# tzt101/MichiGAN

Measured on AMD Instinct MI355X. Metric: training images/sec at 512x512 (G+D step), higher is better.
Workload: dtype bf16; 1 GPU; SPADEB G + multiscale PatchGAN D + VGG19 + Gabor orientation losses, full G step + D step (Adam), bs=8/GPU, 512x512, BASELINE.json configs[2]; global_batch=8, batch_per_gpu=8, resolution=512, parallelism=dp1, init=reference default (xavier, 0.02), random VGG weights

## Files before the change

### michigan_amd/_cabi.py

```python
from __future__ import annotations

import contextlib
import ctypes
import os

MG_F32, MG_BF16 = 0, 1
MG_ACT_NONE, MG_ACT_RELU, MG_ACT_LRELU, MG_ACT_TANH = 0, 1, 2, 3
MG_EPI_PLAIN, MG_EPI_SPADE = 0, 1
MG_MAX_TAPS = 64
MG_ABI_VERSION = 10
MG_COMM_ID_BYTES = 128

OPT_CONV_BIGTILES, OPT_CONV_HALO, OPT_WGRAD3X3, OPT_CONV_HALO_BIG, OPT_CONV_SPLITK, OPT_CONV_THIN, OPT_CONV_WIDE, OPT_CONV_DOT = 1, 2, 3, 4, 5, 6, 7, 8
OPT_PROBE_HALO_VARIANT, OPT_PROBE_WGRAD3X3, OPT_PROBE_ADDR_LO, OPT_PROBE_ADDR_HI, OPT_PROBE_NOXPRE = 10, 12, 13, 14, 15
OPT_WGRAD_MIN_STAGES, OPT_NORM_BWD_VEC, OPT_PROBE_HALO_LDSPAD, OPT_CONV_HALO64, OPT_PROBE_HALO64_DBG, OPT_WGRAD3X3_STRIPE = 18, 19, 21, 22, 23, 24

_i32, _f32, _vp, _i64 = ctypes.c_int32, ctypes.c_float, ctypes.c_void_p, ctypes.c_int64


class ConvDesc(ctypes.Structure):
    _fields_ = [
        ("in_", _vp), ("wt", _vp), ("out", _vp), ("bias", _vp), ("resid", _vp), ("x", _vp),
        ("mean", _vp), ("rstd", _vp), ("gamma_out", _vp),
        ("dtype", _i32), ("N", _i32), ("Hin", _i32), ("Win", _i32), ("Cin", _i32),
# ... 102 lines not shown
    "mg_pixel_affine": ([_vp, _vp, _vp, _vp, _i32, _i64, _i32, _vp, _vp], _i32),
    "mg_bg_compose": ([_vp, _vp, _vp, _i64, _i32, _i32, _i32, _i32, _i32, _i32, _vp, _vp, _vp], _i32),
    "mg_masked_mean_fill": ([_vp, _vp, _vp, _vp, _i32, _i32, _i32, _i32, _vp, _vp], _i32),
    "mg_orient_loss_fwd": ([_vp, _vp, _vp, _i32, _i64, _vp, _i64, _i32, _i64, _vp, _vp, _vp], _i32),
    "mg_orient_loss_bwd": ([_vp, _vp, _vp, _i32, _i64, _vp, _i64, _vp, _vp, _vp, _i32, _i64, _vp, _vp], _i32),
    "mg_color_loss_fwd": ([_vp, _vp, _i64, _vp, _i64, _i32, _i32, _i32, _i32, _i32, _i32, _vp, _vp, _vp], _i32),
    "mg_color_loss_bwd": ([_vp, _vp, _i64, _vp, _i64, _vp, _vp, _vp, _i32, _i32, _i32, _i32, _i32, _i32, _vp, _vp], _i32),
    "mg_hair_lab_fwd": ([_vp, _vp, _i64, _vp, _i64, _vp, _i64, _vp, _i64, _vp, _i64, _i32, _i32, _i32, _i32, _i32, _i32, _vp, _vp, _vp, _vp], _i32),
    "mg_hair_lab_bwd": ([_vp, _vp, _i64, _vp, _i64, _vp, _i64, _vp, _vp, _vp, _i32, _i32, _i32, _i32, _i32, _i32, _vp, _vp], _i32),
    "mg_gabor_argmax_fwd": ([_vp, _vp, _vp, _vp, _i32, _i32, _i32, _i32, _i32, _vp], _i32),
    "mg_gabor_argmax_bwd": ([_vp, _vp, _vp, _vp, _i32, _i32, _i32, _i32, _i32, _vp], _i32),
    "mg_self_attention": ([_vp, _vp, _vp, _vp, _i32, _i32, _i32, _i32, _i32, _i64, _i64, _i64, _i64, _vp], _i32),
    "mg_sn_normalize": ([_vp, _i32, _f32, _vp, _vp, _vp, _vp], _i32),
    "mg_sn_scale": ([_vp, _vp, _vp, _i64, _vp], _i32),
    "mg_sn_bwd": ([_vp, _vp, _vp, _vp, _vp, _vp, _i32, _i32, _vp], _i32),
    "mg_adam_step": ([_vp, _vp, _vp, _vp, _i64, _f32, _f32, _f32, _f32, _i32, _f32, _vp], _i32),
    "mg_input_crop_u8": ([_vp, _vp, _vp, _vp, _vp, _vp, _i32, _i32, _i32, _i32, _i32, _i32, _i32, _i32, _vp], _i32),
    "mg_onehot_labels": ([_vp, _vp, _i32, _i64, _i32, _vp], _i32),
    "mg_orient_to_rgb_u8": ([_vp, _vp, _vp, _vp, _i64, _vp], _i32),
    "mg_generate_hole_u8": ([_vp, _vp, _vp, _vp, _vp, _vp, _i32, _i32, _i32, _vp], _i32),
    "mg_noise_octaves": ([_vp, _vp, _i32, _i32, _vp], _i32),
    "mg_resize_bicubic_u8": ([_vp, _vp, _vp, _vp, _vp, _i32, _vp, _vp, _i32, _i32, _i32, _i32, _i32, _i32, _i32, _vp], _i32),
    "mg_bicubic_ksize": ([_i32, _i32], _i32),
    "mg_inputs_set_option": ([_i32, _i32], _i32),
    "mg_bicubic_table": ([_i32, _i32, _vp, _vp], _i32),
    "mg_nearest_table": ([_i32, _i32, _vp], _i32),
    "mg_orient_rgb_table": ([_vp], _i32),
    "mg_noise_field_len": ([_i32], _i64),
    "mg_comm_unique_id": ([_vp], _i32),
    "mg_comm_init": ([_vp, _i32, _i32, ctypes.POINTER(_i64)], _i32),
    "mg_comm_destroy": ([_i64], _i32),
    "mg_comm_world": ([_i64, ctypes.POINTER(_i32), ctypes.POINTER(_i32)], _i32),
    "mg_allreduce_stats": ([_i64, _vp, _i64, _i32, _vp], _i32),
    "mg_allreduce_grads": ([_i64, _vp, _i64, _vp], _i32),
    "mg_probe_mfma_layout": ([_vp, _vp], _i32),
    "mg_probe_tr16": ([_vp, _vp, _vp], _i32),
    "mg_set_option": ([_i32, _i32], _i32),
    "mg_get_option": ([_i32, ctypes.POINTER(_i32)], _i32),
    "mg_sizeof_desc": ([_i32], _i32),
    "mg_abi_version": ([], _i32),
    "mg_last_error": ([], ctypes.c_char_p),
    "mg_feat_moment_workspace": ([_i32, _i64, _i32], _i64),
    "mg_feat_moment_loss_fwd": ([ctypes.POINTER(FeatMomentDesc), _vp], _i32),
    "mg_feat_moment_loss_bwd": ([ctypes.POINTER(FeatMomentDesc), _vp, _vp, _vp, _vp], _i32),
    "mg_orient_smooth": ([_vp, _vp, _vp, _vp, _vp, _vp, _vp, _i32, _i32, _i32, _vp], _i32),
    "mg_stroke_orient": ([_vp, _vp, _vp, _vp, _vp, _vp, _i32, _i32, _i32, _vp], _i32),
    "mg_stroke_compose": ([_vp, _vp, _vp, _vp, _vp, _vp, _vp, _i32, _i32, _i32, _i32, _i32, _i32, _vp, _vp], _i32),
    "mg_inpaint_finish": ([_vp, _vp, _vp, _vp, _vp, _vp, _i32, _i32, _i32, _i32, _i32, _vp, _vp, _vp], _i32),
}
_EDIT_PROTOS = {
    "mge_brush_u8": ([_vp, _vp, _i32, _i32, _i32, _i32, _vp], _i32),
    "mge_morph_u8": ([_vp, _vp, _i32, _i32, _i32, _i32, _i32, _vp, _i32, _i32, _i32, _vp], _i32),
}
EXPORTED_SYMBOLS = tuple(_PROTOS)
_NO_STATUS = {"mg_wgrad_det_workspace", "mg_norm_apply2_supported", "mg_grad_slot_blocks", "mg_pack_job_blocks", "mg_sn_layer_blocks", "mg_stats_workspace", "mg_sizeof_desc", "mg_abi_version", "mg_last_error", "mg_noise_field_len", "mg_bicubic_ksize",
              "mg_feat_moment_workspace"}
_BY_REF = {fn for fn, (argtypes, _) in _PROTOS.items()
           if argtypes and isinstance(getattr(argtypes[0], "_type_", None), type) and issubclass(argtypes[0]._type_, ctypes.Structure)}
DESC_MIRRORS = (ConvDesc, WgradDesc, GradSlot, PackJob, SnLayer, NormApply2Desc, PyramidDesc, FeatMomentDesc)

LIB_PATH = os.environ.get("MG_LIB") or os.path.join(os.path.dirname(os.path.abspath(__file__)), "lib", "libmichigan_hip.so")


class HipBackend:
    name = "hip"

    def __init__(self, path: str = LIB_PATH):
        if not os.path.exists(path) and path == LIB_PATH and os.environ.get("MG_AUTOBUILD", "1") != "0":
            import sys
            print("[michigan_amd] libmichigan_hip.so missing: building it with hipcc (gfx950), ~2 min", file=sys.stderr, flush=True)
            from . import build as _build
            _build.build_locked(verbose=False)
        if not os.path.exists(path):
            raise RuntimeError(
                f"libmichigan_hip.so not found at {path}: build it with "
                "`python -c 'import __graft_entry__ as g; g.build()'` (hipcc, gfx950). "
                "michigan_amd has no CPU / eager-PyTorch fallback.")
        import torch
        self._lib = ctypes.CDLL(path)
        for fn, (argtypes, restype) in list(_PROTOS.items()) + list(_EDIT_PROTOS.items()):
            f = getattr(self._lib, fn)
            f.argtypes, f.restype = argtypes, restype
        if self._lib.mg_abi_version() != MG_ABI_VERSION:
            raise RuntimeError("libmichigan_hip.so ABI version mismatch")
        if any(self._lib.mg_sizeof_desc(which) != ctypes.sizeof(mirror) for which, mirror in enumerate(DESC_MIRRORS)):
            raise RuntimeError("ctypes mirror of the descriptor structs is out of sync with include/michigan_hip.h")

    def __getattr__(self, fn):
        if fn not in _PROTOS and fn not in _EDIT_PROTOS:
            raise AttributeError(fn)
        raw = getattr(self._lib, fn)
        if fn in _NO_STATUS:
            return raw
        by_ref = fn in _BY_REF

        def call(*args):
            if by_ref:
                args = (ctypes.byref(args[0]),) + tuple(args[1:])
            rc = raw(*args)
            if rc != 0:
                msg = self._lib.mg_last_error()
                raise RuntimeError(f"{fn} failed (code {rc}): {msg.decode() if msg else '?'}")
            return rc
        self.__dict__[fn] = call
        return call


_backend = None


def backend():
    global _backend
    if _backend is None:
        _backend = HipBackend()
    return _backend


def set_backend(obj):
    global _backend
    prev, _backend = _backend, obj
    return prev


def get_option(key, be=None):
    v = _i32()
    (be or backend()).mg_get_option(key, ctypes.byref(v))
    return v.value


@contextlib.contextmanager
def options(values, be=None):
    be = be or backend()
    saved = {key: get_option(key, be) for key in values}
    try:
        for key, v in values.items():
            be.mg_set_option(key, v)
        yield
    finally:
        for key, v in saved.items():
            be.mg_set_option(key, v)
```

### michigan_amd/build.py

```python
from __future__ import annotations

import hashlib
import os
import shutil
import subprocess
import sys
from concurrent.futures import ThreadPoolExecutor

PKG_DIR = os.path.dirname(os.path.abspath(__file__))
REPO_ROOT = os.path.dirname(PKG_DIR)
CSRC = os.path.join(PKG_DIR, "csrc")
INCLUDE = os.path.join(REPO_ROOT, "include")
LIB_DIR = os.path.join(PKG_DIR, "lib")
OBJ_DIR = os.path.join(LIB_DIR, "obj")
LIB_PATH = os.path.join(LIB_DIR, "libmichigan_hip.so")

ARCH = "gfx950"
SOURCES = ["mg_api.hip", "mg_conv.hip", "mg_wgrad.hip", "mg_norm.hip", "mg_pointwise.hip", "mg_pack.hip", "mg_conv_halo.hip", "mg_conv_halo64.hip", "mg_gabor.hip", "mg_wgrad3x3.hip", "mg_spectral.hip", "mg_conv_thin.hip", "mg_inputs.hip", "mg_conv_dot.hip", "mg_loss.hip", "mg_grad.hip", "mg_weights.hip", "mg_glue.hip", "mg_color_loss.hip", "mg_hair_lab.hip", "mg_feat_moments.hip", "mg_orient_smooth.hip", "mg_stroke.hip", "mg_mask_edit.hip", "mg_attention.hip", "mg_comm.hip"]
CXXFLAGS = [f"--offload-arch={ARCH}", "-O3", "-std=c++17", "-fPIC", "-munsafe-fp-atomics",
            "-fno-gpu-rdc", f"-I{INCLUDE}", f"-I{CSRC}"]


def _hipcc() -> str:
    for cand in (os.environ.get("HIPCC"), "/opt/rocm/bin/hipcc", shutil.which("hipcc")):
        if cand and os.path.exists(cand):
            return cand
    raise RuntimeError("hipcc not found (looked at $HIPCC, /opt/rocm/bin/hipcc, PATH)")


def _public_headers() -> list:
    return sorted(os.path.join(d, f) for d, _, files in os.walk(INCLUDE) for f in files)


def _fingerprint(src: str = "") -> str:
    h = hashlib.sha256()
    h.update(" ".join(CXXFLAGS).encode())
    paths = [os.path.join(CSRC, f) for f in sorted(os.listdir(CSRC)) if f.endswith(".h") or (not src and f.endswith(".hip"))]
    paths += _public_headers()
    if src:
        paths.append(os.path.join(CSRC, src))
    for p in paths:
        if os.path.isfile(p):
            h.update(os.path.basename(p).encode())
            with open(p, "rb") as fh:
                h.update(fh.read())
    return h.hexdigest()


def source_hash() -> str:
    h = hashlib.sha256()
    h.update(" ".join(f for f in CXXFLAGS if not f.startswith("-I")).encode())
    for p in [os.path.join(CSRC, f) for f in sorted(os.listdir(CSRC))] + _public_headers():
        if p.endswith((".h", ".hip")):
            h.update(os.path.relpath(p, REPO_ROOT).replace(os.sep, "/").encode())
            with open(p, "rb") as fh:
                h.update(fh.read())
    return h.hexdigest()[:16]


def build(force: bool = False, verbose: bool = True) -> str:
    os.makedirs(OBJ_DIR, exist_ok=True)
    stamp = os.path.join(LIB_DIR, "build.stamp")
    fp = _fingerprint()
    if not force and os.path.exists(LIB_PATH) and os.path.exists(stamp):
        with open(stamp) as fh:
            if fh.read().strip() == fp:
                return LIB_PATH
    hipcc = _hipcc()

    def compile_one(src: str) -> str:
        obj = os.path.join(OBJ_DIR, os.path.splitext(src)[0] + ".o")
# ... 42 lines not shown
```

### michigan_amd/csrc/mg_pointwise.hip

```cpp
#include "mg_common.h"
#include "mg_launch.h"
#include "mg_reduce.h"

namespace {

template <typename T>
__global__ void act_bwd_kernel(const T* __restrict__ dy, const T* __restrict__ y, T* __restrict__ dpre,
                               int64_t nquads, int act, float slope)
{
    MG_GRID_STRIDE(i, nquads) {
        const f32x4_t d = ET<T>::load4(dy + i * 4), v = ET<T>::load4(y + i * 4);
        f32x4_t o;
#pragma unroll
        for (int j = 0; j < 4; ++j) o[j] = d[j] * mg_act_grad_from_out(v[j], act, slope);
        ET<T>::store4(dpre + i * 4, o);
    }
}

template <typename T>
__global__ void up2_fwd_kernel(const T* __restrict__ x, T* __restrict__ y, int N, int H, int W, int C)
{
    const int c4 = C / 4; const int Ho = 2 * H, Wo = 2 * W;
    const int64_t n = (int64_t)N * Ho * Wo * c4;
    MG_GRID_STRIDE(i, n) {
// ... 89 lines not shown
        const float inv = 1.f / (float)(pool_cnt(oy, H) * pool_cnt(ox, W));
#pragma unroll
        for (int j = 0; j < 4; ++j) s[j] *= inv;
        ET<T>::store4(y + i * 4, s);
    }
}
template <typename T>
__global__ void avgpool_bwd_kernel(const T* __restrict__ dy, T* __restrict__ dx, int N, int H, int W, int C, int Ho, int Wo)
{
    const int c4 = C / 4;
    const int64_t n = (int64_t)N * H * W * c4;
    MG_GRID_STRIDE(i, n) {
        const int qd = (int)(i % c4); int64_t p = i / c4;
        const int ix = (int)(p % W); p /= W;
        const int iy = (int)(p % H); const int b = (int)(p / H);
        f32x4_t s = {0.f, 0.f, 0.f, 0.f};
        for (int oy = (iy) >> 1; oy <= (iy + 1) >> 1; ++oy) {
            if (oy >= Ho) continue;
            for (int ox = (ix) >> 1; ox <= (ix + 1) >> 1; ++ox) {
                if (ox >= Wo) continue;
                const float inv = 1.f / (float)(pool_cnt(oy, H) * pool_cnt(ox, W));
                const f32x4_t v = ET<T>::load4(dy + (((size_t)b * Ho + oy) * Wo + ox) * C + qd * 4);
#pragma unroll
                for (int j = 0; j < 4; ++j) s[j] += v[j] * inv;
            }
        }
        ET<T>::store4(dx + i * 4, s);
    }
}

template <typename T>
__global__ void maxpool_fwd_kernel(const T* __restrict__ x, T* __restrict__ y, int N, int H, int W, int C, int Ho, int Wo)
{
    const int c4 = C / 4;
    const int64_t n = (int64_t)N * Ho * Wo * c4;
    MG_GRID_STRIDE(i, n) {
        const int qd = (int)(i % c4); int64_t p = i / c4;
        const int ox = (int)(p % Wo); p /= Wo;
        const int oy = (int)(p % Ho); const int b = (int)(p / Ho);
        const size_t base = (((size_t)b * H + 2 * oy) * W + 2 * ox) * C + qd * 4;
        const f32x4_t a = ET<T>::load4(x + base), bq = ET<T>::load4(x + base + C);
        const f32x4_t c = ET<T>::load4(x + base + (size_t)W * C), e = ET<T>::load4(x + base + (size_t)W * C + C);
        f32x4_t o;
#pragma unroll
        for (int j = 0; j < 4; ++j) o[j] = fmaxf(fmaxf(a[j], bq[j]), fmaxf(c[j], e[j]));
        ET<T>::store4(y + i * 4, o);
    }
}
template <typename T>
__global__ void maxpool_bwd_kernel(const T* __restrict__ dy, const T* __restrict__ x, T* __restrict__ dx,
                                   int N, int H, int W, int C, int Ho, int Wo, int relu_in)
{
    const int c4 = C / 4;
    const int64_t n = (int64_t)N * H * W * c4;
    MG_GRID_STRIDE(i, n) {
        const int qd = (int)(i % c4); int64_t p = i / c4;
        const int ix = (int)(p % W); p /= W;
        const int iy = (int)(p % H); const int b = (int)(p / H);
        const int oy = iy >> 1, ox = ix >> 1;
        f32x4_t o = {0.f, 0.f, 0.f, 0.f};
        if (oy < Ho && ox < Wo) {
            const size_t base = (((size_t)b * H + 2 * oy) * W + 2 * ox) * C + qd * 4;
            f32x4_t v[4];
            v[0] = ET<T>::load4(x + base); v[1] = ET<T>::load4(x + base + C);
            v[2] = ET<T>::load4(x + base + (size_t)W * C); v[3] = ET<T>::load4(x + base + (size_t)W * C + C);
            const f32x4_t g = ET<T>::load4(dy + (((size_t)b * Ho + oy) * Wo + ox) * C + qd * 4);
            const int me = (iy & 1) * 2 + (ix & 1);
#pragma unroll
            for (int j = 0; j < 4; ++j) {
                int arg = 0; float m = v[0][j];
#pragma unroll
                for (int k = 1; k < 4; ++k) if (v[k][j] > m) { m = v[k][j]; arg = k; }
                o[j] = (arg == me && (!relu_in || m > 0.f)) ? g[j] : 0.f;
            }
        }
        ET<T>::store4(dx + i * 4, o);
    }
}

template <typename T>
__global__ void blend_fwd_kernel(const T* __restrict__ bg, const T* __restrict__ x, const float* __restrict__ hair,
                                 const float* __restrict__ back, T* __restrict__ y, int64_t nquads, int C, int act, float slope)
{
    const int c4 = C / 4;
    MG_GRID_STRIDE(i, nquads) {
        const int64_t p = i / c4;
        const float wb = 1.f - hair[p], wx = 1.f - back[p];
        const f32x4_t b = ET<T>::load4(bg + i * 4), v = ET<T>::load4(x + i * 4);
        f32x4_t o;
#pragma unroll
        for (int j = 0; j < 4; ++j) o[j] = mg_act(b[j] * wb + v[j] * wx, act, slope);
        ET<T>::store4(y + i * 4, o);
    }
}
template <typename T>
__global__ void blend_bwd_kernel(const T* __restrict__ dy, const T* __restrict__ y, const float* __restrict__ hair,
                                 const float* __restrict__ back, T* __restrict__ dbg, T* __restrict__ dx, int64_t nquads, int C,
                                 int act, float slope)
{
    const int c4 = C / 4;
    MG_GRID_STRIDE(i, nquads) {
        const int64_t p = i / c4;
        const float wb = 1.f - hair[p], wx = 1.f - back[p];
        f32x4_t d = ET<T>::load4(dy + i * 4);
        if (act != MG_ACT_NONE) {
            const f32x4_t yv = ET<T>::load4(y + i * 4);
#pragma unroll
            for (int j = 0; j < 4; ++j) d[j] *= mg_act_grad_from_out(yv[j], act, slope);
        }
        f32x4_t a, b;
#pragma unroll
        for (int j = 0; j < 4; ++j) { a[j] = d[j] * wb; b[j] = d[j] * wx; }
        if (dbg) ET<T>::store4(dbg + i * 4, a);
        if (dx)  ET<T>::store4(dx + i * 4, b);
    }
}

__global__ void adam_kernel(float* __restrict__ p, const float* __restrict__ g, float* __restrict__ m, float* __restrict__ v,
                            int64_t n, float lr, float b1, float b2, float eps, float bc1, float bc2_sqrt, float gscale)
{
    MG_GRID_STRIDE(i, n) {
        const float gi = g[i] * gscale;
        const float w = 1.f - b1, mo = b1 == 0.f ? 0.f : m[i];
        const float mi = w < 0.5f ? mo + w * (gi - mo) : gi - (gi - mo) * (1.f - w);
        const float vi = v[i] * b2 + gi * gi * (1.f - b2);
        m[i] = mi; v[i] = vi;
        const float denom = sqrtf(vi) / bc2_sqrt + eps;
        p[i] = p[i] - (lr / bc1) * (mi / denom);
    }
// ... 189 lines not shown
        ET<T>::store4(out + (size_t)i * 8 + 4, b);
    }
}

extern "C" int mg_assemble_nhwc8(const float* planar, int32_t cp, const void* nhwc, int32_t cs, int32_t cf, void* out, int32_t dtype,
                                 int32_t N, int64_t HW, void* stream)
{
    MG_CHECK_ARG(out && (planar || cp == 0) && (nhwc || cf == 0), "mg_assemble_nhwc8: null pointer");
    MG_CHECK_ARG((dtype == MG_F32 || dtype == MG_BF16) && N > 0 && HW > 0 && cp >= 0 && cf >= 0 && cp + cf <= 8 && cf <= cs,
                 "mg_assemble_nhwc8: bad geometry (cp + cf <= 8, cf <= cs)");
    hipStream_t st = reinterpret_cast<hipStream_t>(stream);
    const int64_t npix = (int64_t)N * HW;
    mg_by_dtype(dtype, [&](auto t) { using T = typename decltype(t)::type;
        hipLaunchKernelGGL(assemble_nhwc8_kernel<T>, dim3(mg_ew_grid(npix, 8192)), dim3(MG_NTHR), 0, st, planar, cp, (const T*)nhwc, cs, cf, (T*)out, npix, HW); });
    MG_CHECK_LAUNCH("mg_assemble_nhwc8");
    return MG_OK;
}

template <typename T>
__global__ void grad_sum_act_kernel(const T* __restrict__ g1, const T* __restrict__ g2, const T* __restrict__ y, T* __restrict__ out,
                                    int64_t nquads, int act, float slope)
{
    MG_GRID_STRIDE(i, nquads) {
        f32x4_t a = ET<T>::load4(g1 + i * 4);
        if (g2) { const f32x4_t b = ET<T>::load4(g2 + i * 4);
#pragma unroll
            for (int j = 0; j < 4; ++j) a[j] += b[j]; }
        const f32x4_t v = ET<T>::load4(y + i * 4);
#pragma unroll
        for (int j = 0; j < 4; ++j) a[j] *= mg_act_grad_from_out(v[j], act, slope);
        ET<T>::store4(out + i * 4, a);
    }
}

extern "C" int mg_grad_sum_act(const void* g1, const void* g2, const void* y, void* out, int32_t dtype, int64_t numel, int32_t act,
                               float slope, void* stream)
{
    MG_CHECK_ARG(g1 && y && out, "mg_grad_sum_act: null pointer");
    MG_CHECK_ARG((dtype == MG_F32 || dtype == MG_BF16) && numel > 0 && (numel % 4) == 0, "mg_grad_sum_act: numel must be a positive multiple of 4");
    hipStream_t st = reinterpret_cast<hipStream_t>(stream);
    const int64_t nq = numel / 4;
    mg_by_dtype(dtype, [&](auto t) { using T = typename decltype(t)::type;
        hipLaunchKernelGGL(grad_sum_act_kernel<T>, dim3(mg_ew_grid(nq, 8192)), dim3(MG_NTHR), 0, st, (const T*)g1, (const T*)g2, (const T*)y, (T*)out, nq, act, slope); });
    MG_CHECK_LAUNCH("mg_grad_sum_act");
    return MG_OK;
}

extern "C" int mg_maxpool2_bwd(const void* dy, const void* x, void* dx, int32_t dtype, int32_t N, int32_t H, int32_t W, int32_t C, int32_t relu_input, void* stream)
{
    MG_EW_GEOM("mg_maxpool2_bwd"); MG_CHECK_ARG(dy && x && dx, "mg_maxpool2_bwd: null pointer");
    MG_CHECK_ARG(H >= 2 && W >= 2, "mg_maxpool2_bwd: H, W must be >= 2");
    hipStream_t st = reinterpret_cast<hipStream_t>(stream);
    const int Ho = H / 2, Wo = W / 2;
    const int g = mg_ew_grid((int64_t)N * H * W * (C / 4), 8192);
    mg_by_dtype(dtype, [&](auto t) { using T = typename decltype(t)::type;
        hipLaunchKernelGGL(maxpool_bwd_kernel<T>, dim3(g), dim3(MG_NTHR), 0, st, (const T*)dy, (const T*)x, (T*)dx, N, H, W, C, Ho, Wo, relu_input); });
    MG_CHECK_LAUNCH("mg_maxpool2_bwd");
    return MG_OK;
}

extern "C" int mg_blend_fwd(const void* bg, const void* x, const float* hair, const float* back, void* y,
                            int32_t dtype, int64_t P, int32_t C, int32_t act, float slope, void* stream)
{
    MG_CHECK_ARG(bg && x && hair && back && y, "mg_blend_fwd: null pointer");
    MG_CHECK_ARG((dtype == MG_F32 || dtype == MG_BF16) && P > 0 && C > 0 && (C % 4) == 0, "mg_blend_fwd: bad geometry");
    hipStream_t st = reinterpret_cast<hipStream_t>(stream);
    const int64_t nq = P * (C / 4);
    mg_by_dtype(dtype, [&](auto t) { using T = typename decltype(t)::type;
        hipLaunchKernelGGL(blend_fwd_kernel<T>, dim3(mg_ew_grid(nq, 8192)), dim3(MG_NTHR), 0, st, (const T*)bg, (const T*)x, hair, back, (T*)y, nq, C, act, slope); });
    MG_CHECK_LAUNCH("mg_blend_fwd");
    return MG_OK;
}
extern "C" int mg_blend_bwd(const void* dy, const void* y, const float* hair, const float* back, void* dbg, void* dx,
                            int32_t dtype, int64_t P, int32_t C, int32_t act, float slope, void* stream)
{
    MG_CHECK_ARG(dy && hair && back && (dbg || dx) && (y || act == MG_ACT_NONE), "mg_blend_bwd: null pointer");
    MG_CHECK_ARG((dtype == MG_F32 || dtype == MG_BF16) && P > 0 && C > 0 && (C % 4) == 0, "mg_blend_bwd: bad geometry");
    hipStream_t st = reinterpret_cast<hipStream_t>(stream);
    const int64_t nq = P * (C / 4);
    mg_by_dtype(dtype, [&](auto t) { using T = typename decltype(t)::type;
        hipLaunchKernelGGL(blend_bwd_kernel<T>, dim3(mg_ew_grid(nq, 8192)), dim3(MG_NTHR), 0, st, (const T*)dy, (const T*)y, hair, back, (T*)dbg, (T*)dx, nq, C, act, slope); });
    MG_CHECK_LAUNCH("mg_blend_bwd");
    return MG_OK;
}

extern "C" int mg_adam_step(float* param, const float* grad, float* exp_avg, float* exp_avg_sq,
                            int64_t numel, float lr, float beta1, float beta2, float eps, int32_t step,
                            float grad_scale, void* stream)
{
    MG_CHECK_ARG(param && grad && exp_avg && exp_avg_sq, "mg_adam_step: null pointer");
    MG_CHECK_ARG(numel > 0 && step >= 1, "mg_adam_step: bad numel/step");
    hipStream_t st = reinterpret_cast<hipStream_t>(stream);
    const double bc1 = 1.0 - pow((double)beta1, (double)step);
    const double bc2 = 1.0 - pow((double)beta2, (double)step);
    hipLaunchKernelGGL(adam_kernel, dim3(mg_ew_grid(numel, 8192)), dim3(MG_NTHR), 0, st, param, grad, exp_avg, exp_avg_sq, numel,
                       lr, beta1, beta2, eps, (float)bc1, (float)sqrt(bc2), grad_scale);
    MG_CHECK_LAUNCH("mg_adam_step");
    return MG_OK;
}

extern "C" int mg_probe_mfma_layout(float* out, void* stream)
{
    MG_CHECK_ARG(out, "mg_probe_mfma_layout: null pointer");
    hipLaunchKernelGGL(probe_mfma_kernel, dim3(1), dim3(64), 0, reinterpret_cast<hipStream_t>(stream), out);
    MG_CHECK_LAUNCH("mg_probe_mfma_layout");
    return MG_OK;
}
// ... 34 lines not shown
```

### michigan_amd/networks/discriminator.py

```python
from __future__ import annotations

import numpy as np
import torch.nn as nn

from .. import ops
from . import spectral
from .base_network import BaseNetwork
from .layers import HipConv2d
from .normalization import get_nonspade_norm_layer


class NLayerDiscriminator(BaseNetwork):

    @staticmethod
    def modify_commandline_options(parser, is_train):
        parser.add_argument("--n_layers_D", type=int, default=4, help="# layers in each discriminator")
        return parser

    def __init__(self, opt):
        super().__init__()
        self.opt = opt
        kw, padw, nf = 4, int(np.ceil((4 - 1.0) / 2)), opt.ndf
        norm_layer = get_nonspade_norm_layer(opt, opt.norm_D)
        groups = [[HipConv2d(self.compute_D_input_nc(opt), nf, kw, stride=2, padding=padw), nn.LeakyReLU(0.2, False)]]
        for n in range(1, opt.n_layers_D):
            prev, nf = nf, min(nf * 2, 512)
            stride = 1 if n == opt.n_layers_D - 1 else 2
            groups.append([norm_layer(HipConv2d(prev, nf, kw, stride=stride, padding=padw)), nn.LeakyReLU(0.2, False)])
        groups.append([HipConv2d(nf, 1, kw, stride=1, padding=padw)])
        for n, g in enumerate(groups):
            self.add_module("model%d" % n, nn.Sequential(*g))

    def compute_D_input_nc(self, opt):
        nc = opt.label_nc + opt.output_nc + opt.orient_nc
        nc += 1 if opt.contain_dontcare_label else 0
        nc += 0 if opt.no_instance else 1
        return nc

    def forward(self, x):
        feats = []
        groups = list(self.children())
        for i, g in enumerate(groups):
            head, fused_lrelu = g[0], len(g) > 1
            act = ops.ACT_LRELU if fused_lrelu else ops.ACT_NONE
            x = head(x, act=act)
            feats.append(x)
        return feats if not self.opt.no_ganFeat_loss else feats[-1]


class MultiscaleDiscriminator(BaseNetwork):

    @staticmethod
    def modify_commandline_options(parser, is_train):
        parser.add_argument("--netD_subarch", type=str, default="n_layer", help="architecture of each discriminator")
        parser.add_argument("--num_D", type=int, default=2, help="number of discriminators to be used in multiscale")
        opt, _ = parser.parse_known_args()
        if opt.netD_subarch != "n_layer":
            raise ValueError("unrecognized discriminator subarchitecture %s" % opt.netD_subarch)
        NLayerDiscriminator.modify_commandline_options(parser, is_train)
        return parser

    def __init__(self, opt):
        super().__init__()
        self.opt = opt
        for i in range(opt.num_D):
            self.add_module("discriminator_%d" % i, self.create_single_discriminator(opt))

    def create_single_discriminator(self, opt):
        if opt.netD_subarch != "n_layer":
            raise ValueError("unrecognized discriminator subarchitecture %s" % opt.netD_subarch)
        return NLayerDiscriminator(opt)

    def downsample(self, x):
        return ops.avgpool3s2(x)

    def forward(self, input):
        spectral.prepare(self)
        x = ops.pad_channels(ops.to_nhwc(input, self.compute_dtype), 8)
        result = []
        for _, d in self.named_children():
            out = d(x)
            out = [ops.to_nchw(t) for t in out] if isinstance(out, list) else [ops.to_nchw(out)]
            result.append(out)
            x = self.downsample(x)
        return result
```

### michigan_amd/ops.py

```python
from __future__ import annotations

import ctypes
import os
import weakref
from typing import List, Optional, Sequence, Tuple

import torch
import torch.nn.functional as F

from . import _cabi as C

ACT_NONE, ACT_RELU, ACT_LRELU, ACT_TANH = C.MG_ACT_NONE, C.MG_ACT_RELU, C.MG_ACT_LRELU, C.MG_ACT_TANH

WGRAD_USE_TR = True
SYNC_BN_GROUP = None
SYNC_BN_ASYNC = os.environ.get("MG_SYNCBN_ASYNC", "0") == "1"
GRAD_SINK = True
WGRAD_DETERMINISTIC = os.environ.get("MG_DETERMINISTIC") == "1"


def set_deterministic(flag: bool = True) -> bool:
    global WGRAD_DETERMINISTIC
    prev, WGRAD_DETERMINISTIC = WGRAD_DETERMINISTIC, bool(flag)
    return prev
# ... 1209 lines not shown
    return _ReflectPadFn.apply(x, p)


def upsample2x(x):
    y = _Up2Fn.apply(x)
    y._mg_stats_src = x.detach()
    return y


def avgpool3s2(x):
    return _AvgPoolFn.apply(x)


def maxpool2(x):
    return _MaxPoolFn.apply(x, getattr(x, "_mg_relu_out", False))


class _AssembleFn(torch.autograd.Function):

    @staticmethod
    def forward(ctx, image, planar, dst, n0, cf):
        n, h, w, cs = image.shape
        cp = planar.shape[1]
        C.backend().mg_assemble_nhwc8(_p(planar), cp, _p(image), cs, cf, _p(dst[n0:n0 + n]), _dt(dst), n, h * w, _stream(dst))
        ctx.meta = (n0, n, cp, cf, cs)
        ctx.mark_dirty(dst)
        return dst

    @staticmethod
    def backward(ctx, g):
        n0, n, cp, cf, cs = ctx.meta
        dimg = g[n0:n0 + n, :, :, cp:cp + cf]
        if cs != cf:
            dimg = F.pad(dimg, (0, cs - cf))
        return dimg.contiguous(), None, None, None, None


def assemble_nhwc8(dst: torch.Tensor, n0: int, planar: torch.Tensor, image: Optional[torch.Tensor] = None, cf: int = 0) -> torch.Tensor:
    planar = planar.detach().float().contiguous()
    if image is None:
        n, _, h, w = planar.shape
        C.backend().mg_assemble_nhwc8(_p(planar), planar.shape[1], None, 0, 0, _p(dst[n0:n0 + n]), _dt(dst), n, h * w, _stream(dst))
        return dst
    image = _nhwc(image)
    if image.dtype != dst.dtype:
        image = image.to(dst.dtype)
    if image.requires_grad and torch.is_grad_enabled():
        return _AssembleFn.apply(image, planar, dst, n0, cf)
    n, h, w, cs = image.shape
    C.backend().mg_assemble_nhwc8(_p(planar), planar.shape[1], _p(image), cs, cf, _p(dst[n0:n0 + n]), _dt(dst), n, h * w, _stream(dst))
    return dst


class _ActTapFn(torch.autograd.Function):

    @staticmethod
    def forward(ctx, a, act, slope):
        ctx.save_for_backward(a)
        ctx.cfg = (act, slope)
        return a.view_as(a), a.view_as(a)

    @staticmethod
    def backward(ctx, g1, g2):
        (a,) = ctx.saved_tensors
        act, slope = ctx.cfg
        if g1 is None and g2 is None:
            return None, None, None
        if g1 is None:
            g1, g2 = g2, None
        g1 = g1.contiguous()
        _take_mask_record(g1, a)
        if g2 is not None:
            g2 = g2.contiguous()
            _take_mask_record(g2, a)
        out = torch.empty_like(a)
        C.backend().mg_grad_sum_act(_p(g1), _p(g2), _p(a), _p(out), _dt(a), a.numel(), act, slope, _stream(a))
        if act == ACT_RELU:
            _leave_mask_record(out, a)
        return out, None, None


def act_tap(a: torch.Tensor, act: int = ACT_RELU, slope: float = 0.2):
    if act != ACT_RELU or not (torch.is_grad_enabled() and a.requires_grad) or a.numel() % 4 or not FUSE_RELU_MASK:
        return a, a
    a1, a2 = _ActTapFn.apply(a, act, slope)
    a1._mg_relu_out = a2._mg_relu_out = getattr(a, "_mg_relu_out", False)
    return a1, a2


def blend(bg, x, hair_mask, back_mask, *, act: int = ACT_NONE, slope: float = 0.2):
    return _BlendFn.apply(bg, x, hair_mask, back_mask, act, slope)


class _L1MeanFn(torch.autograd.Function):
    @staticmethod
    def forward(ctx, a, b):
        if a.shape != b.shape or a.dtype != b.dtype:
            raise ValueError("l1_mean: tensors must agree in shape and dtype")
        n = a.numel()
        out = torch.empty(1, dtype=torch.float32, device=a.device)
        ws = torch.empty(1024, dtype=torch.float32, device=a.device)
        C.backend().mg_l1_mean_fwd(_p(a), _p(b), _dt(a), n, _p(out), _p(ws), _stream(a))
        ctx.save_for_backward(a, b)
        return out.reshape(())

    @staticmethod
    def backward(ctx, g):
        a, b = ctx.saved_tensors
        g = g.reshape(1).float().contiguous()
        da = torch.empty_like(a)
        C.backend().mg_l1_mean_bwd(_p(a), _p(b), _p(g), _dt(a), a.numel(), _p(da), _stream(a))
        return da, None


class _L1HalvesFn(torch.autograd.Function):

    @staticmethod
    def forward(ctx, t):
        half = t.shape[0] // 2
        a, b = t[:half], t[half:]
        out = torch.empty(1, dtype=torch.float32, device=t.device)
        ws = torch.empty(1024, dtype=torch.float32, device=t.device)
        C.backend().mg_l1_mean_fwd(_p(a), _p(b), _dt(t), a.numel(), _p(out), _p(ws), _stream(t))
        ctx.save_for_backward(t)
        return out.reshape(())

    @staticmethod
    def backward(ctx, g):
        (t,) = ctx.saved_tensors
        half = t.shape[0] // 2
        g = g.reshape(1).float().contiguous()
        dt = torch.empty_like(t)
        C.backend().mg_l1_mean_bwd(_p(t[:half]), _p(t[half:]), _p(g), _dt(t), t[:half].numel(), _p(dt[:half]), _stream(t))
        dt[half:].zero_()
        return dt


def l1_mean_halves(t: torch.Tensor) -> torch.Tensor:
    t = _dense_view(t)
    half = t.shape[0] // 2
    if t.shape[0] % 2 or t[:half].numel() % 4 or t.dtype not in (torch.float32, torch.bfloat16):
        return F.l1_loss(t[:half].float(), t[half:].detach().float())
    return _L1HalvesFn.apply(t)


def _dense_view(t: torch.Tensor) -> torch.Tensor:
    if t.dim() == 4:
        v = t.permute(0, 2, 3, 1)
        if v.is_contiguous():
            return v
    return t.contiguous()


def l1_mean(a: torch.Tensor, b: torch.Tensor) -> torch.Tensor:
    a, b = _dense_view(a), _dense_view(b.detach())
    if a.dtype != b.dtype:
        b = b.to(a.dtype)
    if a.numel() % 4 or a.dtype not in (torch.float32, torch.bfloat16):
        return F.l1_loss(a.float(), b.float())
    return _L1MeanFn.apply(a, b)


def _plane_args(t: torch.Tensor):
    if t.dtype != torch.float32 or t.dim() != 3 or t.stride(2) != 1 or t.stride(1) != t.shape[2]:
        raise ValueError("expected an fp32 [N, H, W] view with dense rows")
    return t.data_ptr(), (t.stride(0) if t.shape[0] > 1 else t.shape[1] * t.shape[2])


def planes_of(t: torch.Tensor):
    t = t.detach()
    if t.dtype != torch.float32:
        t = t.float()
    if not t.is_contiguous():
        t = t.contiguous()
    return [t[:, c] for c in range(t.shape[1])]


def nearest_pyramid(planes, sizes, cout: int, dtype):
    n, H, W = planes[0].shape
    if not (1 <= len(planes) <= 8 and len(planes) <= cout <= 8 and 1 <= len(sizes) <= 8):
        raise ValueError("nearest_pyramid: at most 8 planes / channels / levels")
    d = C.PyramidDesc()
    for c, pl in enumerate(planes):
        if pl.shape != planes[0].shape or pl.device != planes[0].device:
            raise ValueError("nearest_pyramid: planes disagree in shape / device")
        d.plane[c], d.nstride[c] = _plane_args(pl)
    d.nplanes, d.N, d.H, d.W, d.nlev, d.cout = len(planes), n, H, W, len(sizes), cout
    outs = []
    d.dtype = _dtype_code(dtype)
    for l, (h, w) in enumerate(sizes):
        o = torch.empty((n, int(h), int(w), cout), dtype=dtype, device=planes[0].device)
        d.h[l], d.w[l], d.out[l] = int(h), int(w), o.data_ptr()
        outs.append(o)
    C.backend().mg_nearest_pyramid(d, _stream(planes[0]))
    return outs


def pconv_mask(mask: torch.Tensor, k: int, s: int, p: int):
    m = mask.detach()
    if m.dim() == 4:
        m = m.reshape(m.shape[0], m.shape[1], m.shape[2]) if m.shape[3] == 1 else m[:, 0]
    m = m.float().contiguous()
    n, H, W = m.shape
    h, w = (H + 2 * p - k) // s + 1, (W + 2 * p - k) // s + 1
    scale = torch.empty((n, h, w, 1), dtype=torch.float32, device=m.device)
    upd = torch.empty((n, h, w, 1), dtype=torch.float32, device=m.device)
    C.backend().mg_pconv_mask(_p(m), n, H, W, k, s, p, _p(scale), _p(upd), _stream(m))
    return scale, upd


class _PixelAffineFn(torch.autograd.Function):
    @staticmethod
    def forward(ctx, x, a, bias, b):
# ... 754 lines not shown
```

Before: 132.5 images/s.

## Fuse L1 loss backward into activation tap backward and scatter maxpool gradients

Adds a fused kernel that computes the L1-mean gradient, adds it to the incoming gradient and applies the activation derivative in one pass. L1 loss nodes that hang off an activation or feature tap now only record the gradient scale, and the tap's backward runs the fused kernel. This drops separate da buffers, zero fills and add kernels for VGG and discriminator feature-matching losses. Maxpool backward is also rewritten to iterate over output positions and write each 2x2 window directly, which cuts redundant input loads. The autograd coupling between nodes is intricate and could misorder or drop gradients if the graph shape differs from what is expected.

```diff
diff --git a/include/michigan_hip/loss_taps.h b/include/michigan_hip/loss_taps.h
--- /dev/null
+++ b/include/michigan_hip/loss_taps.h
@@ -0,0 +1,16 @@
+#ifndef MICHIGAN_HIP_LOSS_TAPS_H
+#define MICHIGAN_HIP_LOSS_TAPS_H
+
+#include "../michigan_hip.h"
+
+#ifdef __cplusplus
+extern "C" {
+#endif
+
+int mgl_tap_l1_bwd(const void* g_in, const void* a, const void* b, const float* gscale, const void* y, void* out, int32_t dtype,
+                   int64_t numel, int64_t n_l1, int32_t act, float slope, void* stream);
+
+#ifdef __cplusplus
+}
+#endif
+#endif
diff --git a/michigan_amd/_cabi.py b/michigan_amd/_cabi.py
--- a/michigan_amd/_cabi.py
+++ b/michigan_amd/_cabi.py
@@ -178,6 +178,10 @@
     "mge_brush_u8": ([_vp, _vp, _i32, _i32, _i32, _i32, _vp], _i32),
     "mge_morph_u8": ([_vp, _vp, _i32, _i32, _i32, _i32, _i32, _vp, _i32, _i32, _i32, _vp], _i32),
 }
+_LOSS_TAP_PROTOS = {
+    "mgl_tap_l1_bwd": ([_vp, _vp, _vp, _vp, _vp, _vp, _i32, _i64, _i64, _i32, _f32, _vp], _i32),
+}
+_EXT_PROTOS = {**_EDIT_PROTOS, **_LOSS_TAP_PROTOS}
 EXPORTED_SYMBOLS = tuple(_PROTOS)
 _NO_STATUS = {"mg_wgrad_det_workspace", "mg_norm_apply2_supported", "mg_grad_slot_blocks", "mg_pack_job_blocks", "mg_sn_layer_blocks", "mg_stats_workspace", "mg_sizeof_desc", "mg_abi_version", "mg_last_error", "mg_noise_field_len", "mg_bicubic_ksize",
               "mg_feat_moment_workspace"}
@@ -204,7 +208,7 @@
                 "michigan_amd has no CPU / eager-PyTorch fallback.")
         import torch
         self._lib = ctypes.CDLL(path)
-        for fn, (argtypes, restype) in list(_PROTOS.items()) + list(_EDIT_PROTOS.items()):
+        for fn, (argtypes, restype) in list(_PROTOS.items()) + list(_EXT_PROTOS.items()):
             f = getattr(self._lib, fn)
             f.argtypes, f.restype = argtypes, restype
         if self._lib.mg_abi_version() != MG_ABI_VERSION:
@@ -213,7 +217,7 @@
             raise RuntimeError("ctypes mirror of the descriptor structs is out of sync with include/michigan_hip.h")
 
     def __getattr__(self, fn):
-        if fn not in _PROTOS and fn not in _EDIT_PROTOS:
+        if fn not in _PROTOS and fn not in _EXT_PROTOS:
             raise AttributeError(fn)
         raw = getattr(self._lib, fn)
         if fn in _NO_STATUS:
@@ -246,6 +250,10 @@
     global _backend
     prev, _backend = _backend, obj
     return prev
+
+
+def has_loss_taps(be=None) -> bool:
+    return getattr(be or backend(), "mgl_tap_l1_bwd", None) is not None
 
 
 def get_option(key, be=None):
diff --git a/michigan_amd/build.py b/michigan_amd/build.py
--- a/michigan_amd/build.py
+++ b/michigan_amd/build.py
@@ -16,7 +16,7 @@
 LIB_PATH = os.path.join(LIB_DIR, "libmichigan_hip.so")
 
 ARCH = "gfx950"
-SOURCES = ["mg_api.hip", "mg_conv.hip", "mg_wgrad.hip", "mg_norm.hip", "mg_pointwise.hip", "mg_pack.hip", "mg_conv_halo.hip", "mg_conv_halo64.hip", "mg_gabor.hip", "mg_wgrad3x3.hip", "mg_spectral.hip", "mg_conv_thin.hip", "mg_inputs.hip", "mg_conv_dot.hip", "mg_loss.hip", "mg_grad.hip", "mg_weights.hip", "mg_glue.hip", "mg_color_loss.hip", "mg_hair_lab.hip", "mg_feat_moments.hip", "mg_orient_smooth.hip", "mg_stroke.hip", "mg_mask_edit.hip", "mg_attention.hip", "mg_comm.hip"]
+SOURCES = ["mg_api.hip", "mg_conv.hip", "mg_wgrad.hip", "mg_norm.hip", "mg_pointwise.hip", "mg_pack.hip", "mg_conv_halo.hip", "mg_conv_halo64.hip", "mg_gabor.hip", "mg_wgrad3x3.hip", "mg_spectral.hip", "mg_conv_thin.hip", "mg_inputs.hip", "mg_conv_dot.hip", "mg_loss.hip", "mg_grad.hip", "mg_weights.hip", "mg_glue.hip", "mg_color_loss.hip", "mg_hair_lab.hip", "mg_feat_moments.hip", "mg_orient_smooth.hip", "mg_stroke.hip", "mg_mask_edit.hip", "mg_loss_taps.hip", "mg_attention.hip", "mg_comm.hip"]
 CXXFLAGS = [f"--offload-arch={ARCH}", "-O3", "-std=c++17", "-fPIC", "-munsafe-fp-atomics",
             "-fno-gpu-rdc", f"-I{INCLUDE}", f"-I{CSRC}"]
 
diff --git a/michigan_amd/csrc/mg_loss_taps.hip b/michigan_amd/csrc/mg_loss_taps.hip
--- /dev/null
+++ b/michigan_amd/csrc/mg_loss_taps.hip
@@ -0,0 +1,96 @@
+#include "mg_common.h"
+#include "mg_launch.h"
+#include "michigan_hip/loss_taps.h"
+#include <type_traits>
+
+namespace {
+
+template <typename T> __device__ __forceinline__ float tap_round(float v)
+{
+    if constexpr (std::is_same<T, float>::value) return v; else return bf2f(f2bf(v));
+}
+
+template <typename T, bool WIDE> struct TapVec {
+    static constexpr int V = WIDE ? EV<T>::VEC : 4;
+    __device__ static __forceinline__ void load(const T* p, float (&v)[V])
+    {
+        if constexpr (WIDE) EV<T>::load(p, v);
+        else { const f32x4_t t = ET<T>::load4(p); v[0] = t[0]; v[1] = t[1]; v[2] = t[2]; v[3] = t[3]; }
+    }
+    __device__ static __forceinline__ void store(T* p, const float (&v)[V])
+    {
+        if constexpr (WIDE) EV<T>::store(p, v);
+        else ET<T>::store4(p, f32x4_t{v[0], v[1], v[2], v[3]});
+    }
+};
+
+template <typename T, bool WIDE>
+__global__ __launch_bounds__(MG_NTHR) void tap_l1_bwd_kernel(const T* g_in, const T* __restrict__ a, const T* __restrict__ b,
+                                                             const float* __restrict__ gscale, float inv_n, const T* __restrict__ y,
+                                                             T* out, int64_t nvec, int64_t nvec_l1, int act, float slope)
+{
+    using IO = TapVec<T, WIDE>;
+    constexpr int V = IO::V;
+    const float s = gscale[0] * inv_n;
+    const float sp = tap_round<T>(s), sn = tap_round<T>(-s);
+    MG_GRID_STRIDE(i, nvec) {
+        float u[V];
+        if (i < nvec_l1) {
+            float p[V], q[V];
+            IO::load(a + i * V, p); IO::load(b + i * V, q);
+#pragma unroll
+            for (int j = 0; j < V; ++j) { const float d = p[j] - q[j]; u[j] = d > 0.f ? sp : (d < 0.f ? sn : 0.f); }
+        } else {
+#pragma unroll
+            for (int j = 0; j < V; ++j) u[j] = 0.f;
+        }
+        if (g_in) {
+            float g[V];
+            IO::load(g_in + i * V, g);
+#pragma unroll
+            for (int j = 0; j < V; ++j) u[j] = g[j] + u[j];
+        }
+        if (act != MG_ACT_NONE) {
+            float v[V];
+            IO::load(y + i * V, v);
+#pragma unroll
+            for (int j = 0; j < V; ++j) u[j] *= mg_act_grad_from_out(v[j], act, slope);
+        }
+        IO::store(out + i * V, u);
+    }
+}
+
+inline bool tap_disjoint(const void* p, int64_t pbytes, const void* q, int64_t qbytes)
+{
+    const char* a = (const char*)p; const char* b = (const char*)q;
+    return !a || !b || a + pbytes <= b || b + qbytes <= a;
+}
+
+}
+
+extern "C" int mgl_tap_l1_bwd(const void* g_in, const void* a, const void* b, const float* gscale, const void* y, void* out, int32_t dtype,
+                              int64_t numel, int64_t n_l1, int32_t act, float slope, void* stream)
+{
+    MG_CHECK_ARG(a && b && gscale && out, "mgl_tap_l1_bwd: null pointer");
+    MG_CHECK_ARG(dtype == MG_F32 || dtype == MG_BF16, "mgl_tap_l1_bwd: dtype must be MG_F32 or MG_BF16");
+    MG_CHECK_ARG(act == MG_ACT_NONE || act == MG_ACT_RELU || act == MG_ACT_LRELU, "mgl_tap_l1_bwd: act must be NONE, RELU or LRELU");
+    MG_CHECK_ARG(y || act == MG_ACT_NONE, "mgl_tap_l1_bwd: an activation needs its output y");
+    MG_CHECK_ARG(numel > 0 && n_l1 > 0 && n_l1 <= numel && (numel % 4) == 0 && (n_l1 % 4) == 0,
+                 "mgl_tap_l1_bwd: 0 < n_l1 <= numel, both multiples of 4 (got %lld, %lld)", (long long)n_l1, (long long)numel);
+    const int64_t esz = dtype == MG_BF16 ? 2 : 4, bytes = numel * esz, l1_bytes = n_l1 * esz;
+    MG_CHECK_ARG(tap_disjoint(out, bytes, a, l1_bytes) && tap_disjoint(out, bytes, b, l1_bytes) && tap_disjoint(out, bytes, y, bytes)
+                 && tap_disjoint(out, bytes, gscale, 4) && (g_in == out || tap_disjoint(out, bytes, g_in, bytes)),
+                 "mgl_tap_l1_bwd: out overlaps an input (only out == g_in is an in-place form)");
+    hipStream_t st = reinterpret_cast<hipStream_t>(stream);
+    const int64_t vec = 16 / esz;
+    const uintptr_t low = (uintptr_t)g_in | (uintptr_t)a | (uintptr_t)b | (uintptr_t)y | (uintptr_t)out;
+    const bool wide = (low & 15) == 0 && (numel % vec) == 0 && (n_l1 % vec) == 0;
+    const int64_t per = wide ? vec : 4, nvec = numel / per, nvec_l1 = n_l1 / per;
+    const float inv_n = (float)(1.0 / (double)n_l1);
+    mg_by_dtype(dtype, [&](auto t) { using T = typename decltype(t)::type;
+        mg_by_bool(wide, [&](auto w) {
+            hipLaunchKernelGGL((tap_l1_bwd_kernel<T, decltype(w)::value>), dim3(mg_ew_grid(nvec, 8192)), dim3(MG_NTHR), 0, st,
+                               (const T*)g_in, (const T*)a, (const T*)b, gscale, inv_n, (const T*)y, (T*)out, nvec, nvec_l1, act, slope); }); });
+    MG_CHECK_LAUNCH("mgl_tap_l1_bwd");
+    return MG_OK;
+}
diff --git a/michigan_amd/csrc/mg_pointwise.hip b/michigan_amd/csrc/mg_pointwise.hip
--- a/michigan_amd/csrc/mg_pointwise.hip
+++ b/michigan_amd/csrc/mg_pointwise.hip
@@ -165,29 +165,35 @@
                                    int N, int H, int W, int C, int Ho, int Wo, int relu_in)
 {
     const int c4 = C / 4;
-    const int64_t n = (int64_t)N * H * W * c4;
-    MG_GRID_STRIDE(i, n) {
-        const int qd = (int)(i % c4); int64_t p = i / c4;
-        const int ix = (int)(p % W); p /= W;
-        const int iy = (int)(p % H); const int b = (int)(p / H);
-        const int oy = iy >> 1, ox = ix >> 1;
-        f32x4_t o = {0.f, 0.f, 0.f, 0.f};
-        if (oy < Ho && ox < Wo) {
-            const size_t base = (((size_t)b * H + 2 * oy) * W + 2 * ox) * C + qd * 4;
-            f32x4_t v[4];
-            v[0] = ET<T>::load4(x + base); v[1] = ET<T>::load4(x + base + C);
-            v[2] = ET<T>::load4(x + base + (size_t)W * C); v[3] = ET<T>::load4(x + base + (size_t)W * C + C);
-            const f32x4_t g = ET<T>::load4(dy + (((size_t)b * Ho + oy) * Wo + ox) * C + qd * 4);
-            const int me = (iy & 1) * 2 + (ix & 1);
-#pragma unroll
-            for (int j = 0; j < 4; ++j) {
-                int arg = 0; float m = v[0][j];
-#pragma unroll
-                for (int k = 1; k < 4; ++k) if (v[k][j] > m) { m = v[k][j]; arg = k; }
-                o[j] = (arg == me && (!relu_in || m > 0.f)) ? g[j] : 0.f;
-            }
-        }
-        ET<T>::store4(dx + i * 4, o);
+    const int64_t n = (int64_t)N * Ho * Wo * c4;
+    const size_t row = (size_t)W * C;
+    MG_GRID_STRIDE(i, n) {
+        const int qd = (int)(i % c4); int64_t p = i / c4;
+        const int ox = (int)(p % Wo); p /= Wo;
+        const int oy = (int)(p % Ho); const int b = (int)(p / Ho);
+        const size_t base = (((size_t)b * H + 2 * oy) * W + 2 * ox) * C + qd * 4;
+        f32x4_t v[4], o[4];
+        v[0] = ET<T>::load4(x + base); v[1] = ET<T>::load4(x + base + C);
+        v[2] = ET<T>::load4(x + base + row); v[3] = ET<T>::load4(x + base + row + C);
+        const f32x4_t g = ET<T>::load4(dy + i * 4);
+#pragma unroll
+        for (int j = 0; j < 4; ++j) {
+            int arg = 0; float m = v[0][j];
+#pragma unroll
+            for (int k = 1; k < 4; ++k) if (v[k][j] > m) { m = v[k][j]; arg = k; }
+            const bool keep = !relu_in || m > 0.f;
+#pragma unroll
+            for (int k = 0; k < 4; ++k) o[k][j] = (arg == k && keep) ? g[j] : 0.f;
+        }
+        ET<T>::store4(dx + base, o[0]); ET<T>::store4(dx + base + C, o[1]);
+        ET<T>::store4(dx + base + row, o[2]); ET<T>::store4(dx + base + row + C, o[3]);
+        const f32x4_t z = {0.f, 0.f, 0.f, 0.f};
+        const bool ex = (W & 1) && ox == Wo - 1, ey = (H & 1) && oy == Ho - 1;
+        if (ex) { ET<T>::store4(dx + base + 2 * (size_t)C, z); ET<T>::store4(dx + base + row + 2 * (size_t)C, z); }
+        if (ey) {
+            ET<T>::store4(dx + base + 2 * row, z); ET<T>::store4(dx + base + 2 * row + C, z);
+            if (ex) ET<T>::store4(dx + base + 2 * row + 2 * (size_t)C, z);
+        }
     }
 }
 
@@ -483,7 +489,7 @@
     MG_CHECK_ARG(H >= 2 && W >= 2, "mg_maxpool2_bwd: H, W must be >= 2");
     hipStream_t st = reinterpret_cast<hipStream_t>(stream);
     const int Ho = H / 2, Wo = W / 2;
-    const int g = mg_ew_grid((int64_t)N * H * W * (C / 4), 8192);
+    const int g = mg_ew_grid((int64_t)N * Ho * Wo * (C / 4), 8192);
     mg_by_dtype(dtype, [&](auto t) { using T = typename decltype(t)::type;
         hipLaunchKernelGGL(maxpool_bwd_kernel<T>, dim3(g), dim3(MG_NTHR), 0, st, (const T*)dy, (const T*)x, (T*)dx, N, H, W, C, Ho, Wo, relu_input); });
     MG_CHECK_LAUNCH("mg_maxpool2_bwd");
diff --git a/michigan_amd/networks/discriminator.py b/michigan_amd/networks/discriminator.py
--- a/michigan_amd/networks/discriminator.py
+++ b/michigan_amd/networks/discriminator.py
@@ -44,7 +44,10 @@
             head, fused_lrelu = g[0], len(g) > 1
             act = ops.ACT_LRELU if fused_lrelu else ops.ACT_NONE
             x = head(x, act=act)
-            feats.append(x)
+            feat = x
+            if i < len(groups) - 1 and not self.opt.no_ganFeat_loss:
+                x, feat = ops.feature_tap(x)
+            feats.append(feat)
         return feats if not self.opt.no_ganFeat_loss else feats[-1]
 
 
diff --git a/michigan_amd/ops.py b/michigan_amd/ops.py
--- a/michigan_amd/ops.py
+++ b/michigan_amd/ops.py
@@ -1285,22 +1285,76 @@
     return dst
 
 
+FUSE_L1_TAP = os.environ.get("MG_FUSE_L1_TAP", "1") != "0"
+_VIEW_NODES = ("PermuteBackward0", "ViewBackward0", "UnsafeViewBackward0", "AliasBackward0", "TransposeBackward0")
+
+
+class _L1Record:
+    __slots__ = ("b", "n", "gscale")
+
+    def __init__(self, b, n):
+        self.b, self.n, self.gscale = b, n, None
+
+
+def _tap_of(t: torch.Tensor):
+    if not (FUSE_L1_TAP and torch.is_grad_enabled() and t.requires_grad and t.is_contiguous() and C.has_loss_taps()):
+        return None
+    fn = t.grad_fn
+    for _ in range(4):
+        if fn is None or isinstance(fn, _ActTapFn._backward_cls):
+            break
+        if fn.name() not in _VIEW_NODES or len(fn.next_functions) != 1:
+            return None
+        fn = fn.next_functions[0][0]
+    if not isinstance(fn, _ActTapFn._backward_cls) or getattr(fn, "tap_key", None) != (t.data_ptr(), t.numel(), t.dtype):
+        return None
+    return fn
+
+
 class _ActTapFn(torch.autograd.Function):
 
     @staticmethod
     def forward(ctx, a, act, slope):
         ctx.save_for_backward(a)
         ctx.cfg = (act, slope)
+        ctx.tap_key = (a.data_ptr(), a.numel(), a.dtype) if a.is_contiguous() else None
+        ctx.l1 = []
+        ctx.set_materialize_grads(False)
         return a.view_as(a), a.view_as(a)
 
     @staticmethod
     def backward(ctx, g1, g2):
         (a,) = ctx.saved_tensors
         act, slope = ctx.cfg
-        if g1 is None and g2 is None:
-            return None, None, None
+        due = [(r, r.gscale) for r in ctx.l1 if r.gscale is not None]
+        for r, _ in due:
+            r.gscale = None
         if g1 is None:
             g1, g2 = g2, None
+        if len(due) == 1 and g2 is None and (g1 is None or (g1.shape == a.shape and g1.dtype == a.dtype)) and C.has_loss_taps():
+            (r, gs), = due
+            g1 = None if g1 is None else g1.contiguous()
+            if g1 is not None:
+                _take_mask_record(g1, a)
+            out = torch.empty_like(a)
+            C.backend().mgl_tap_l1_bwd(_p(g1), _p(a), _p(r.b), _p(gs), _p(a) if act != ACT_NONE else None, _p(out), _dt(a),
+                                       a.numel(), r.n, act, slope, _stream(a))
+            if act == ACT_RELU:
+                _leave_mask_record(out, a)
+            return out, None, None
+        for r, gs in due:
+            da = torch.empty_like(a)
+            C.backend().mg_l1_mean_bwd(_p(a), _p(r.b), _p(gs), _dt(a), r.n, _p(da), _stream(a))
+            if r.n < a.numel():
+                da.view(-1)[r.n:].zero_()
+            if g1 is None:
+                g1 = da
+            else:
+                g2 = da if g2 is None else g2 + da
+        if g1 is None:
+            return None, None, None
+        if act == ACT_NONE:
+            return (g1 if g2 is None else g1 + g2), None, None
         g1 = g1.contiguous()
         _take_mask_record(g1, a)
         if g2 is not None:
@@ -1321,52 +1375,82 @@
     return a1, a2
 
 
+def feature_tap(x: torch.Tensor):
+    if not (FUSE_L1_TAP and torch.is_grad_enabled() and x.requires_grad and x.is_contiguous() and x.numel() % 4 == 0
+            and x.dtype in (torch.float32, torch.bfloat16) and C.has_loss_taps()):
+        return x, x
+    return _ActTapFn.apply(x, ACT_NONE, 0.0)
+
+
 def blend(bg, x, hair_mask, back_mask, *, act: int = ACT_NONE, slope: float = 0.2):
     return _BlendFn.apply(bg, x, hair_mask, back_mask, act, slope)
 
 
 class _L1MeanFn(torch.autograd.Function):
-    @staticmethod
-    def forward(ctx, a, b):
+
+    @staticmethod
+    def forward(ctx, a, b, tap):
         if a.shape != b.shape or a.dtype != b.dtype:
             raise ValueError("l1_mean: tensors must agree in shape and dtype")
         n = a.numel()
         out = torch.empty(1, dtype=torch.float32, device=a.device)
         ws = torch.empty(1024, dtype=torch.float32, device=a.device)
         C.backend().mg_l1_mean_fwd(_p(a), _p(b), _dt(a), n, _p(out), _p(ws), _stream(a))
-        ctx.save_for_backward(a, b)
+        ctx.set_materialize_grads(False)
+        ctx.rec = None
+        if tap is not None:
+            ctx.rec = _L1Record(b, n)
+            tap.l1.append(ctx.rec)
+        else:
+            ctx.save_for_backward(a, b)
         return out.reshape(())
 
     @staticmethod
     def backward(ctx, g):
+        if g is None:
+            return None, None, None
+        g = g.reshape(1).float().contiguous()
+        if ctx.rec is not None:
+            ctx.rec.gscale = g
+            return None, None, None
         a, b = ctx.saved_tensors
-        g = g.reshape(1).float().contiguous()
         da = torch.empty_like(a)
         C.backend().mg_l1_mean_bwd(_p(a), _p(b), _p(g), _dt(a), a.numel(), _p(da), _stream(a))
-        return da, None
+        return da, None, None
 
 
 class _L1HalvesFn(torch.autograd.Function):
 
     @staticmethod
-    def forward(ctx, t):
+    def forward(ctx, t, tap):
         half = t.shape[0] // 2
         a, b = t[:half], t[half:]
         out = torch.empty(1, dtype=torch.float32, device=t.device)
         ws = torch.empty(1024, dtype=torch.float32, device=t.device)
         C.backend().mg_l1_mean_fwd(_p(a), _p(b), _dt(t), a.numel(), _p(out), _p(ws), _stream(t))
-        ctx.save_for_backward(t)
+        ctx.set_materialize_grads(False)
+        ctx.rec = None
+        if tap is not None:
+            ctx.rec = _L1Record(b, a.numel())
+            tap.l1.append(ctx.rec)
+        else:
+            ctx.save_for_backward(t)
         return out.reshape(())
 
     @staticmethod
     def backward(ctx, g):
+        if g is None:
+            return None, None
+        g = g.reshape(1).float().contiguous()
+        if ctx.rec is not None:
+            ctx.rec.gscale = g
+            return None, None
         (t,) = ctx.saved_tensors
         half = t.shape[0] // 2
-        g = g.reshape(1).float().contiguous()
         dt = torch.empty_like(t)
         C.backend().mg_l1_mean_bwd(_p(t[:half]), _p(t[half:]), _p(g), _dt(t), t[:half].numel(), _p(dt[:half]), _stream(t))
         dt[half:].zero_()
-        return dt
+        return dt, None
 
 
 def l1_mean_halves(t: torch.Tensor) -> torch.Tensor:
@@ -1374,7 +1458,7 @@
     half = t.shape[0] // 2
     if t.shape[0] % 2 or t[:half].numel() % 4 or t.dtype not in (torch.float32, torch.bfloat16):
         return F.l1_loss(t[:half].float(), t[half:].detach().float())
-    return _L1HalvesFn.apply(t)
+    return _L1HalvesFn.apply(t, _tap_of(t))
 
 
 def _dense_view(t: torch.Tensor) -> torch.Tensor:
@@ -1391,7 +1475,7 @@
         b = b.to(a.dtype)
     if a.numel() % 4 or a.dtype not in (torch.float32, torch.bfloat16):
         return F.l1_loss(a.float(), b.float())
-    return _L1MeanFn.apply(a, b)
+    return _L1MeanFn.apply(a, b, _tap_of(a))
 
 
 def _plane_args(t: torch.Tensor):
```

After: 132.8 images/s (median of 4 runs). Within noise of the previous version (+0.2%).
